# amzn/pecos

Measured on NVIDIA H100. Metric: XR-Linear top-10 queries/sec, higher is better.
Workload: dtype f32

## Files before the change

### pecos_b200/csrc/xlinear_cm_kernel.cuh

```cuda
#pragma once

constexpr int kCmFeat = 8;
constexpr int kCmSlots = 4;
constexpr int kCmMaxWarps = 16;
constexpr int kCmMinWarps = 4;
constexpr uint32_t kCmMaxDup = 400;
constexpr uint32_t kCmSmemBudget = 224u << 10;
constexpr uint32_t kCmMinReuse = 24;
constexpr uint32_t kCmMinPairsPerSm = 48u;
constexpr uint32_t kCmDirectRows = 16384;
constexpr uint32_t kCmEmpty = 0xFFFFFFFFu;

struct CmWork {
    uint32_t* slot_pos;
    uint32_t* count;
    uint32_t* bucket_ptr;
    uint64_t* cost_ptr;
    uint32_t* pair_q;
    uint32_t* pair_pos;
    uint32_t* claim;
    uint32_t* active;
};

struct CmPlan {
// ... 146 lines not shown
            b = rp[r];
            e = rp[r + 1];
            while (b < e && ent[b].x < lo) ++b;
            uint32_t t = b;
            while (t < e && ent[t].x < hi) ++t;
            e = t;
        }
        const uint32_t len = e - b;
        s_scan[threadIdx.x] = len;
        __syncthreads();
        for (uint32_t d = 1; d < 256u; d <<= 1) {
            const uint32_t v = (threadIdx.x >= d) ? s_scan[threadIdx.x - d] : 0u;
            __syncthreads();
            s_scan[threadIdx.x] += v;
            __syncthreads();
        }
        const uint32_t base = s_carry + s_scan[threadIdx.x] - len;
        if (r < R) {
            for (uint32_t i = 0; i < len; ++i) {
                const uint2 en = ent[b + i];
                ec[base + i] = static_cast<unsigned char>(en.x - lo);
                ew[base + i] = __uint_as_float(en.y);
            }
            if (S.direct) {
                unsigned short* starts = reinterpret_cast<unsigned short*>(img + S.off_lookup);
                const uint32_t w_rows = S.words - 1u;
                const uint32_t f = min(ridx[r], w_rows);
                for (uint32_t g = r ? min(ridx[r - 1], w_rows) + 1u : 0u; g <= f; ++g) starts[g] = static_cast<unsigned short>(base);
                if (r + 1u == R)
                    for (uint32_t g = f + 1u; g <= w_rows; ++g) starts[g] = static_cast<unsigned short>(base + len);
            } else {
                rps[r] = static_cast<unsigned short>(base);
            }
            if (r + 1u == R) {
                if (!S.direct) rps[R] = static_cast<unsigned short>(base + len);
                hdr[0] = (h.has_bias & 1u) ? (base | ((base + len) << 16)) : 0u;
                hdr[3] = base + len;
            }
        }
        __syncthreads();
        if (threadIdx.x == 255u) s_carry += s_scan[255];
        __syncthreads();
    }
    if (threadIdx.x == 0) {
        hdr[1] = hi - lo;
        hdr[2] = R;
    }
}

constexpr uint32_t kCmBinWindow = 8192;
constexpr int kCmBucketThreads = 1024;
constexpr uint32_t kCmBucketCtasPerSm = 2;

inline uint32_t cm_bucket_grid(uint32_t rows, uint32_t n_sm) {
    return std::max(1u, std::min(kCmBucketCtasPerSm * n_sm, (rows + kCmBucketThreads / 32 - 1) / (kCmBucketThreads / 32)));
}

struct CmSlotRanges { uint32_t v0, lo, hi, cw; };
__device__ __forceinline__ CmSlotRanges cm_slot_ranges(const uint4 h, const uint32_t* __restrict__ vc_ptr, uint32_t p,
                                                       uint32_t b0, uint32_t nb) {
    CmSlotRanges s{0, 0, 0, 0};
    if ((h.w & kChunkAbsent) || h.y == 0) return s;
    const uint32_t v0 = vc_ptr[p], nr = vc_ptr[p + 1] - v0;
    if (nr == 0) return s;
    s.v0 = v0;
    s.cw = (h.y + nr - 1u) / nr;
    const uint32_t n = min(nr, (h.y + s.cw - 1u) / s.cw);
    s.lo = max(v0, b0);
    s.hi = max(s.lo, min(v0 + n, b0 + nb));
    return s;
}

__device__ __forceinline__ uint2 cm_bucket_block(uint32_t rows) {
    const uint32_t per = (rows + gridDim.x - 1) / gridDim.x;
    const uint32_t b = min(rows, blockIdx.x * per);
    return make_uint2(b, min(rows, b + per));
}

__global__ void __launch_bounds__(kCmBucketThreads, kCmBucketCtasPerSm)
xl_cm_count_kernel(const LayerDev L, const uint32_t* __restrict__ beam_id, const uint32_t* __restrict__ beam_cnt,
                   const uint32_t beam_stride, const uint32_t rows, CmWork w, const uint32_t* __restrict__ vc_ptr,
                   const uint32_t n_vc) {
    __shared__ uint32_t bins[kCmBinWindow];
    const int lane = threadIdx.x & 31, warp = threadIdx.x >> 5, warps = blockDim.x >> 5;
    const uint2 blk = cm_bucket_block(rows);
    for (uint32_t b0 = 0; b0 < n_vc; b0 += kCmBinWindow) {
        const uint32_t nb = min(kCmBinWindow, n_vc - b0);
        for (uint32_t i = threadIdx.x; i < nb; i += blockDim.x) bins[i] = 0u;
        __syncthreads();
        for (uint32_t q = blk.x + warp; q < blk.y; q += warps) {
            const uint32_t cnt = beam_cnt[q];
            uint32_t run = 0;
            for (uint32_t j0 = 0; j0 < cnt; j0 += 32) {
                const uint32_t j = j0 + lane;
                uint4 h = make_uint4(0, 0, 0, kChunkAbsent);
                uint32_t p = 0;
                if (j < cnt) {
                    p = beam_id[static_cast<uint64_t>(q) * beam_stride + j];
                    h = *reinterpret_cast<const uint4*>(&L.chunks[p]);
                }
                if (b0 == 0) {
                    const uint32_t width = (j < cnt) ? h.y : 0u;
                    const uint32_t incl = warp_incl_scan(width, lane);
                    if (j < cnt) w.slot_pos[static_cast<uint64_t>(q) * beam_stride + j] = run + incl - width;
                    run += __shfl_sync(kFull, incl, 31);
                }
                const CmSlotRanges s = cm_slot_ranges(h, vc_ptr, p, b0, nb);
                for (uint32_t v = s.lo; v < s.hi; ++v) atomicAdd(&bins[v - b0], 1u);
            }
        }
        __syncthreads();
        for (uint32_t i = threadIdx.x; i < nb; i += blockDim.x)
            if (bins[i]) atomicAdd(&w.count[b0 + i], bins[i]);
        __syncthreads();
    }
}

__device__ __forceinline__ uint32_t cm_pair_cost(uint32_t w_rows, uint32_t entries) { return w_rows + entries; }

__device__ __forceinline__ uint64_t warp_incl_scan64(uint64_t v, int lane) {
#pragma unroll
    for (int d = 1; d < 32; d <<= 1) {
        const uint64_t t = __shfl_up_sync(kFull, v, d);
        if (lane >= d) v += t;
    }
    return v;
}

__global__ void __launch_bounds__(1024)
xl_cm_scan_kernel(const uint32_t n_chunks, CmWork w, const unsigned char* __restrict__ images, const uint32_t img_bytes,
                  const uint32_t w_rows) {
    __shared__ uint32_t s_pairs[32];
    __shared__ uint64_t s_cost[32];
    __shared__ uint32_t carry_pairs;
    __shared__ uint64_t carry_cost;
    const int lane = threadIdx.x & 31, warp = threadIdx.x >> 5;
    if (threadIdx.x == 0) { carry_pairs = 0; carry_cost = 0; }
    __syncthreads();
    for (uint32_t c0 = 0; c0 < n_chunks; c0 += 1024) {
        const uint32_t c = c0 + threadIdx.x;
        const uint32_t n = (c < n_chunks) ? w.count[c] : 0u;
        const uint32_t unit = n ? cm_pair_cost(w_rows, reinterpret_cast<const uint32_t*>(images + static_cast<uint64_t>(c) * img_bytes)[3]) : 1u;
        const uint64_t cost = static_cast<uint64_t>(n) * unit;
        const uint32_t in_p = warp_incl_scan(n, lane);
        const uint64_t in_c = warp_incl_scan64(cost, lane);
        if (lane == 31) { s_pairs[warp] = in_p; s_cost[warp] = in_c; }
        __syncthreads();
        if (warp == 0) {
            const uint32_t a = s_pairs[lane];
            const uint64_t b = s_cost[lane];
            const uint32_t ia = warp_incl_scan(a, lane);
            const uint64_t ib = warp_incl_scan64(b, lane);
            s_pairs[lane] = ia - a;
            s_cost[lane] = ib - b;
        }
        __syncthreads();
        const uint32_t ex_p = carry_pairs + s_pairs[warp] + in_p - n;
        const uint64_t ex_c = carry_cost + s_cost[warp] + in_c - cost;
        if (c < n_chunks) {
            w.bucket_ptr[c] = ex_p;
            w.cost_ptr[c] = ex_c;
            w.count[c] = ex_p;
            w.claim[c] = ex_p;
            w.active[c] = 0;
        }
        __syncthreads();
        if (threadIdx.x == 1023) { carry_pairs = ex_p + n; carry_cost = ex_c + cost; }
        __syncthreads();
    }
    if (threadIdx.x == 0) { w.bucket_ptr[n_chunks] = carry_pairs; w.cost_ptr[n_chunks] = carry_cost; }
}

__global__ void __launch_bounds__(kCmBucketThreads, kCmBucketCtasPerSm)
xl_cm_scatter_kernel(const LayerDev L, const uint32_t* __restrict__ beam_id, const uint32_t* __restrict__ beam_cnt,
                     const uint32_t beam_stride, const uint32_t rows, CmWork w, const uint32_t* __restrict__ vc_ptr,
                     const uint32_t n_vc) {
    __shared__ uint32_t bins[kCmBinWindow];
    const int lane = threadIdx.x & 31, warp = threadIdx.x >> 5, warps = blockDim.x >> 5;
    const uint2 blk = cm_bucket_block(rows);
    for (uint32_t b0 = 0; b0 < n_vc; b0 += kCmBinWindow) {
        const uint32_t nb = min(kCmBinWindow, n_vc - b0);
        auto each_pair = [&](auto visit) {
            for (uint32_t q = blk.x + warp; q < blk.y; q += warps) {
                const uint32_t cnt = beam_cnt[q];
                for (uint32_t j = lane; j < cnt; j += 32) {
                    const uint32_t p = beam_id[static_cast<uint64_t>(q) * beam_stride + j];
                    const CmSlotRanges s = cm_slot_ranges(*reinterpret_cast<const uint4*>(&L.chunks[p]), vc_ptr, p, b0, nb);
                    if (s.lo < s.hi) visit(q, j, s);
                }
            }
        };
        for (uint32_t i = threadIdx.x; i < nb; i += blockDim.x) bins[i] = 0u;
        __syncthreads();
        each_pair([&](uint32_t, uint32_t, const CmSlotRanges& s) {
            for (uint32_t v = s.lo; v < s.hi; ++v) atomicAdd(&bins[v - b0], 1u);
        });
        __syncthreads();
        for (uint32_t i = threadIdx.x; i < nb; i += blockDim.x)
            if (bins[i]) bins[i] = atomicAdd(&w.count[b0 + i], bins[i]);
        __syncthreads();
        each_pair([&](uint32_t q, uint32_t j, const CmSlotRanges& s) {
            const uint32_t pos = w.slot_pos[static_cast<uint64_t>(q) * beam_stride + j];
            for (uint32_t v = s.lo; v < s.hi; ++v) {
                const uint32_t at = atomicAdd(&bins[v - b0], 1u);
                w.pair_q[at] = q;
                w.pair_pos[at] = pos + (v - s.v0) * s.cw;
            }
        });
        __syncthreads();
    }
}

__device__ inline uint32_t cm_start_chunk(const CmWork& w, uint32_t n_vc, uint32_t b, uint32_t shares) {
    const uint64_t T = w.cost_ptr[n_vc];
    if (T == 0) return n_vc;
    const uint64_t t = static_cast<uint64_t>(T / shares) * b + (T % shares) * b / shares;
    uint32_t lo = 0, hi = n_vc;
    while (hi - lo > 1) {
        const uint32_t mid = (lo + hi) >> 1;
        if (w.cost_ptr[mid] <= t) lo = mid; else hi = mid;
    }
    return lo;
}

enum { kCmPhSwitch, kCmPhCopy, kCmPhStaging, kCmPhLookup, kCmPhAccumulate, kCmPhSlice, kCmPhases };
#ifdef PB200_CM_TRACE
constexpr uint32_t kCmTraceCtas = 1024;
constexpr uint32_t kCmTraceWarp = kCmPhases + 4;
constexpr uint32_t kCmTraceCta = 3 + kCmMaxWarps * kCmTraceWarp;
__device__ unsigned long long g_cm_trace[3 + kCmTraceCtas * kCmTraceCta];
__device__ __forceinline__ unsigned long long cm_globaltimer() {
    unsigned long long t;
    asm volatile("mov.u64 %0, %%globaltimer;" : "=l"(t));
    return t;
}
struct CmTrace {
    unsigned long long start;
    long long t, ph[kCmPhases];
    unsigned long long trips, slots;
    unsigned long long slices, pairs, images;
    __device__ void begin() {
        start = cm_globaltimer();
        t = clock64();
        for (int p = 0; p < kCmPhases; ++p) ph[p] = 0;
        trips = slots = slices = pairs = images = 0;
    }
    __device__ void slice(uint32_t n_pairs) {
        ++slices;
        pairs += n_pairs;
    }
    __device__ void staged() { ++images; }
    __device__ void mark(int p) {
        const long long n = clock64();
        ph[p] += n - t;
        t = n;
    }
    __device__ void count(uint32_t n_trips, uint32_t n_slots) {
        trips += n_trips;
        slots += n_slots;
    }
    __device__ void flush(int warp, int lane, uint32_t launch_pairs) {
        __syncthreads();
        if (blockIdx.x >= kCmTraceCtas) return;
        unsigned long long* rec = g_cm_trace + 3 + blockIdx.x * kCmTraceCta;
        if (threadIdx.x == 0) {
            if (blockIdx.x == 0) { g_cm_trace[0] = gridDim.x; g_cm_trace[1] = blockDim.x >> 5; g_cm_trace[2] = launch_pairs; }
            rec[0] = start;
            rec[1] = cm_globaltimer();
            rec[2] = images;
        }
        for (int d = 16; d > 0; d >>= 1) slots += __shfl_xor_sync(kFull, slots, d);
        if (lane == 0) {
            unsigned long long* wr = rec + 3 + warp * kCmTraceWarp;
            for (int p = 0; p < kCmPhases; ++p) wr[p] = static_cast<unsigned long long>(ph[p]);
            wr[kCmPhases] = trips;
            wr[kCmPhases + 1] = slots;
            wr[kCmPhases + 2] = slices;
            wr[kCmPhases + 3] = pairs;
        }
    }
};
#else
struct CmTrace {
    __device__ void begin() {}
    __device__ void mark(int) {}
    __device__ void count(uint32_t, uint32_t) {}
    __device__ void slice(uint32_t) {}
    __device__ void staged() {}
    __device__ void flush(int, int, uint32_t) {}
};
#endif

template <bool DIRECT, int STAGES, bool PREFIX = false>
__global__ void __launch_bounds__(kCmMaxWarps * 32, 1)
xl_cm_scores_kernel(const LayerDev L, const QueryDev X, const CmWork w, const CmShape S, const unsigned char* __restrict__ images,
                    float* __restrict__ cand, const uint64_t cand_stride_q, const CmPrefixOut P) {
    extern __shared__ __align__(128) unsigned char smem_raw[];
    unsigned char* img = smem_raw;
    const uint32_t* __restrict__ hdr_s = reinterpret_cast<const uint32_t*>(img);
    const unsigned short* __restrict__ start_s = reinterpret_cast<const unsigned short*>(img + S.off_lookup);
    const uint32_t* __restrict__ look_s = reinterpret_cast<const uint32_t*>(img + S.off_lookup);
    const unsigned short* __restrict__ pre_s = reinterpret_cast<const unsigned short*>(img + S.off_pre);
    const unsigned short* __restrict__ rp_s = reinterpret_cast<const unsigned short*>(img + S.off_rp);
    const float* __restrict__ ew_s = reinterpret_cast<const float*>(img + S.off_ew);
    const unsigned char* __restrict__ ec_s = img + S.off_ec;
    const int lane = threadIdx.x & 31;
    const int warp = threadIdx.x >> 5;
    const int nwarps = blockDim.x >> 5;
    constexpr int kStride = kCmFeat + 1;
    constexpr int kBuf = 32 * kStride;
    constexpr int kNBuf = static_cast<int>(cm_buffers(STAGES));
    unsigned char* mine = smem_raw + S.img_bytes + static_cast<size_t>(warp) * cm_warp_bytes(S.acc_cols, STAGES);
    uint32_t* st_idx = reinterpret_cast<uint32_t*>(mine);
    float* st_val = reinterpret_cast<float*>(st_idx + kNBuf * kBuf);
    float* my_acc = st_val + kNBuf * kBuf + lane;

    __shared__ __align__(8) unsigned long long s_mbar;
    const uint32_t mbar = static_cast<uint32_t>(__cvta_generic_to_shared(&s_mbar));
    if (threadIdx.x == 0) {
        cm_mbar_init(mbar, 1u);
        asm volatile("fence.proxy.async.shared::cta;" ::: "memory");
    }
    __syncthreads();
    CmTrace trace;
    trace.begin();

    constexpr int kPerIter = 32 / kCmFeat;
    constexpr int kIters = 32 / kPerIter;
    const int sub = lane / kCmFeat, fl = lane % kCmFeat;
    uint32_t parity = 0;

    uint32_t e = 0, ee = 0, backlog = 0;
    float x = 0.0f;
    uint32_t hp = 0, l1_end = 0;
    auto add_rows = [&](uint32_t row, uint32_t cnt, uint32_t n_ent, bool drain) {
        const uint32_t l2_end = row + cnt;
        const uint32_t avail = backlog + n_ent;
        const uint32_t trips = __reduce_max_sync(kFull, ((drain ? avail : backlog) + kCmSlots - 1u) / kCmSlots);
        if (hp == l1_end) hp = row;
        uint32_t next_r = st_idx[hp];
        float next_x = st_val[hp];
        for (uint32_t t = 0; t < trips; ++t) {
            uint32_t es[kCmSlots], cs[kCmSlots];
            float xs[kCmSlots], a[kCmSlots];
            bool on[kCmSlots];
#pragma unroll
            for (int u = 0; u < kCmSlots; ++u) {
                if (e == ee && hp != l2_end) {
                    e = next_r & 0xFFFFu;
                    ee = next_r >> 16;
                    x = next_x;
                    ++hp;
                    if (hp == l1_end) hp = row;
                    next_r = st_idx[hp];
                    next_x = st_val[hp];
                }
                on[u] = e < ee;
                es[u] = e;
                xs[u] = x;
                e += on[u] ? 1u : 0u;
            }
#pragma unroll
            for (int u = 0; u < kCmSlots; ++u) cs[u] = ec_s[es[u]];
#pragma unroll
            for (int u = 0; u < kCmSlots; ++u) a[u] = my_acc[cs[u] * 32u];
#pragma unroll
            for (int u = 0; u < kCmSlots; ++u) {
                float sum = a[u];
#pragma unroll
                for (int p = 0; p < u; ++p) sum = (cs[p] == cs[u]) ? a[p] : sum;
                a[u] = __fadd_rn(sum, __fmul_rn(xs[u], ew_s[es[u]]));
            }
#pragma unroll
            for (int u = 0; u < kCmSlots; ++u)
                if (on[u]) my_acc[cs[u] * 32u] = a[u];
        }
        const uint32_t added = min(avail, trips * kCmSlots);
        backlog = avail - added;
        trace.count(trips, added);
        l1_end = l2_end;
    };

    uint32_t bias_range = 0, n_cols = 0;
    auto stage_image = [&](uint32_t c) {
        if (threadIdx.x == 0) cm_bulk_load(static_cast<uint32_t>(__cvta_generic_to_shared(img)), images + static_cast<uint64_t>(c) * S.img_bytes, S.img_bytes, mbar);
        cm_mbar_wait(mbar, parity);
        parity ^= 1u;
        trace.staged();
        trace.mark(kCmPhCopy);
        bias_range = hdr_s[0];
        n_cols = hdr_s[1];
    };

    auto score_slice = [&](uint32_t s0, uint32_t s_end) {
        const uint32_t pidx = s0 + lane;
        const bool have = pidx < s_end;
        uint32_t q = 0, pos = 0, qn = 0;
        uint64_t qb = 0;
        if (have) {
            if constexpr (PREFIX) {
                q = pidx;
// ... 218 lines not shown
```

### pecos_b200/csrc/xlinear_engine.cu

```cuda
#include "xlinear_engine.h"
#include "shard_merge.cuh"

#include <algorithm>
#include <atomic>
#include <cstring>
#include <exception>
#include <thread>

namespace pb200 {

namespace {

constexpr unsigned kFull = 0xFFFFFFFFu;
constexpr int kWarpsMax = 10;
constexpr int kMCap = 256;
constexpr int kMFlush = 128;
constexpr int kCSmem = 128;
constexpr int kQCap = 1024;
constexpr int kSortCap = 2048;
constexpr int kTopkThreads = 256;

constexpr int kMCapLookup = 256;

template <int MCAP>
struct __align__(16) WarpScratch {
    uint32_t ms[MCAP];
    float mx[MCAP];
    uint32_t off[MCAP + 4];
    float out[kCSmem];
};

__device__ __forceinline__ uint4 ld_stream_u4(const uint32_t* p) {
    uint4 r;
    asm volatile("ld.global.nc.L1::no_allocate.v4.u32 {%0,%1,%2,%3}, [%4];"
                 : "=r"(r.x), "=r"(r.y), "=r"(r.z), "=r"(r.w) : "l"(p));
    return r;
}

__device__ __forceinline__ int lower_bound_u32(const uint32_t* a, int n, uint32_t key) {
    int lo = 0, hi = n;
    while (lo < hi) {
        int mid = (lo + hi) >> 1;
        if (a[mid] < key) lo = mid + 1; else hi = mid;
    }
    return lo;
}

__device__ __forceinline__ int last_le_u32(const uint32_t* a, int n, uint32_t key) {
    int lo = 0, hi = n;
    while (hi - lo > 1) {
        int mid = (lo + hi) >> 1;
        if (a[mid] <= key) lo = mid; else hi = mid;
    }
    return lo;
}

__device__ __forceinline__ uint32_t warp_incl_scan(uint32_t v, int lane) {
#pragma unroll
    for (int d = 1; d < 32; d <<= 1) {
        uint32_t t = __shfl_up_sync(kFull, v, d);
        if (lane >= d) v += t;
    }
    return v;
}

__device__ __forceinline__ int xl_rows_of_group(const uint32_t* off, int m, uint32_t G, int& row_first, int lane) {
    const int r = row_first + 1 + lane;
    uint32_t bit = 0;
    if (r < m) {
        const uint32_t p = off[r] - G;
        if (p < 32u) bit = 1u << p;
    }
    const uint32_t starts = __reduce_or_sync(kFull, bit);
    const int my_row = row_first + __popc(starts & (0xFFFFFFFFu >> (31 - lane)));
    const int r31 = __shfl_sync(kFull, my_row, 31);
    row_first = (off[r31 + 1] == G + 32u) ? r31 + 1 : r31;
    return my_row;
}

template <int MCAP>
__device__ __forceinline__ void xl_flush_impl(WarpScratch<MCAP>& ws, int m, const uint2* __restrict__ ext,
                                              const uint2* __restrict__ ent, float* out, int lane,
                                              unsigned long long& e_total) {
    if (m == 0) return;
    __syncwarp();
    constexpr int PER = MCAP / 32;
    uint32_t c[PER];
    uint32_t local = 0;
    bool empty_row = false;
#pragma unroll
// ... 288 lines not shown
        }
        __syncwarp();
        if (in_smem) {
            for (uint32_t c = lane; c < h.n_cols; c += 32) blk[c] = ws.out[c];
        }
        __syncwarp();
        if (STATS) { st_chunks += 1; st_rows += R; st_match += m_total; st_ent += e_total; st_cols += h.n_cols; }
    }
    if (STATS) {
        if (lane == 0 && st_chunks) {
            atomicAdd(&stats[0], st_chunks);
            atomicAdd(&stats[1], st_rows);
            atomicAdd(&stats[2], st_match);
            atomicAdd(&stats[3], st_ent);
            atomicAdd(&stats[4], st_cols);
        }
        if (threadIdx.x == 0 && cnt > 0) atomicAdd(&stats[5], static_cast<unsigned long long>(DENSE ? X.cols : qn));
    }
}

__device__ __forceinline__ double xl_hinge_pow(float v, int p) {
    const double zd = fmax(0.0, 1.0 - static_cast<double>(v));
    const float z = static_cast<float>(zd);
    const double x = static_cast<double>(z);
    switch (p) {
        case 0: return 1.0;
        case 1: return x;
        case 2: return x * x;
        case 3: return (x * x) * x;
        case 4: { const double x2 = x * x; return x2 * x2; }
        default: return pow(x, static_cast<double>(static_cast<size_t>(static_cast<long long>(p))));
    }
}

__device__ __forceinline__ float xl_transform(float v, int kind, int p) {
    switch (kind) {
        case PP_SIGMOID: {
            const float e = static_cast<float>(exp(static_cast<double>(-v)));
            return static_cast<float>(1.0 / (1.0 + static_cast<double>(e)));
        }
        case PP_LOG_SIGMOID: {
            const float e = static_cast<float>(exp(static_cast<double>(-v)));
            return static_cast<float>(-log(1.0 + static_cast<double>(e)));
        }
        case PP_LP_HINGE: return static_cast<float>(exp(-xl_hinge_pow(v, p)));
        case PP_LOG_LP_HINGE: return static_cast<float>(-xl_hinge_pow(v, p));
        default: return v;
    }
}

__device__ __forceinline__ float xl_combine(float x, float parent, int kind) {
    switch (kind) {
        case PP_SIGMOID:
        case PP_LP_HINGE: return __fmul_rn(x, parent);
        case PP_LOG_SIGMOID:
        case PP_LOG_LP_HINGE: return __fadd_rn(x, parent);
        default: return x;
    }
}

__device__ __forceinline__ unsigned long long xl_make_key(float v, uint32_t pos) {
    uint32_t u = __float_as_uint(v);
    if ((u & 0x7FFFFFFFu) == 0u) u = 0u;
    u = (u & 0x80000000u) ? ~u : (u | 0x80000000u);
    return (static_cast<unsigned long long>(u) << 32) | static_cast<unsigned long long>(0xFFFFFFFFu - pos);
}

__device__ __forceinline__ unsigned long long xl_exact_key(float v, uint32_t pos) {
    uint32_t u = __float_as_uint(v);
    const uint32_t neg_zero = (u == 0x80000000u) ? 1u : 0u;
    if ((u & 0x7FFFFFFFu) == 0u) u = 0u;
    u = (u & 0x80000000u) ? ~u : (u | 0x80000000u);
    return (static_cast<unsigned long long>(u) << 32) | static_cast<unsigned long long>(0xFFFFFFFFu - ((pos << 1) | neg_zero));
}
__device__ __forceinline__ uint32_t xl_exact_key_pos(unsigned long long key) {
    return (0xFFFFFFFFu - static_cast<uint32_t>(key & 0xFFFFFFFFull)) >> 1;
}
__device__ __forceinline__ float xl_exact_key_value(unsigned long long key) {
    const uint32_t hi = static_cast<uint32_t>(key >> 32);
    const uint32_t bits = (hi & 0x80000000u) ? (hi ^ 0x80000000u) : ~hi;
    return __uint_as_float(((0xFFFFFFFFu - static_cast<uint32_t>(key & 0xFFFFFFFFull)) & 1u) ? 0x80000000u : bits);
}

#include "xlinear_qw_kernel.cuh"
#include "xlinear_cm_kernel.cuh"

__device__ void xl_bitonic_desc(unsigned long long* a, uint32_t n) {
    for (uint32_t k = 2; k <= n; k <<= 1) {
        for (uint32_t j = k >> 1; j > 0; j >>= 1) {
            for (uint32_t i = threadIdx.x; i < n; i += blockDim.x) {
                const uint32_t ixj = i ^ j;
                if (ixj > i) {
                    const unsigned long long x = a[i], y = a[ixj];
                    const bool desc_block = ((i & k) == 0);
                    if (desc_block ? (x < y) : (x > y)) { a[i] = y; a[ixj] = x; }
                }
            }
            __syncthreads();
        }
    }
}

__device__ __forceinline__ uint32_t next_pow2_u32(uint32_t v) {
    if (v <= 2) return 2;
    return 1u << (32 - __clz(v - 1));
}

__global__ void __launch_bounds__(kTopkThreads)
xl_topk_kernel(const LayerDev L, const int pp_kind, const int pp_p, const int combine, const uint32_t k,
               const uint32_t* __restrict__ beam_id, const float* __restrict__ beam_val,
               const uint32_t* __restrict__ beam_cnt, const uint32_t beam_stride, const float* __restrict__ cand,
               const uint64_t cand_stride_q, const uint32_t c_stride, uint32_t* __restrict__ out_id,
               float* __restrict__ out_val, uint32_t* __restrict__ out_cnt, const uint32_t out_stride,
               unsigned long long* sortbuf, const uint64_t sortbuf_stride, const uint32_t b_prev,
               unsigned long long* stats, unsigned long long* __restrict__ out_key) {
    extern __shared__ __align__(16) unsigned char smem_raw[];
    unsigned long long* keys = reinterpret_cast<unsigned long long*>(smem_raw);
    uint32_t* s_base = reinterpret_cast<uint32_t*>(smem_raw + kSortCap * 8);
    uint32_t* s_colbeg = s_base + (b_prev + 1);
    float* s_pval = reinterpret_cast<float*>(s_colbeg + b_prev);

    const uint32_t q = blockIdx.x;
    const uint32_t cnt = beam_cnt[q];
    for (uint32_t j = threadIdx.x; j < cnt; j += blockDim.x) {
        const uint32_t p = beam_id[static_cast<uint64_t>(q) * beam_stride + j];
        const ChunkHeader h = L.chunks[p];
        s_base[j + 1] = h.n_cols;
        s_colbeg[j] = (h.has_bias & kChunkAbsent) ? 0xFFFFFFFFu : h.col_begin;
        s_pval[j] = beam_val[static_cast<uint64_t>(q) * beam_stride + j];
    }
    __syncthreads();
    __shared__ uint32_t s_owned;
    if (threadIdx.x == 0) {
        uint32_t run = 0, owned = 0;
        s_base[0] = 0;
        for (uint32_t j = 0; j < cnt; ++j) {
            if (s_colbeg[j] != 0xFFFFFFFFu) owned += s_base[j + 1];
            run += s_base[j + 1];
            s_base[j + 1] = run;
        }
        s_owned = owned;
    }
    __syncthreads();
    const uint32_t n_valid = s_base[cnt];
    const uint32_t kk = min(k, s_owned);
    if (threadIdx.x == 0) {
        out_cnt[q] = kk;
        if (stats) atomicAdd(&stats[6], static_cast<unsigned long long>(kk));
    }
    if (n_valid == 0) return;

    const float* cq = cand + static_cast<uint64_t>(q) * cand_stride_q;
    auto score_at = [&](uint32_t cpos, uint32_t& label) -> float {
        const uint32_t j = static_cast<uint32_t>(last_le_u32(s_base, static_cast<int>(cnt), cpos));
        const uint32_t off = cpos - s_base[j];
        float v = xl_transform(cq[cpos], pp_kind, pp_p);
        if (combine) v = xl_combine(v, s_pval[j], pp_kind);
        label = s_colbeg[j] + off;
        return v;
    };
    auto key_at = [&](uint32_t cpos) -> unsigned long long {
        const uint32_t j = static_cast<uint32_t>(last_le_u32(s_base, static_cast<int>(cnt), cpos));
        if (s_colbeg[j] == 0xFFFFFFFFu) return 0ull;
        uint32_t lab;
        return xl_make_key(score_at(cpos, lab), cpos);
    };
// ... 529 lines not shown
        b_prev = plan[d].k_cap;
    }
    return plan;
}

uint32_t XLinearEngine::ensure_workspace_(const std::vector<LayerPlan>& plan, uint32_t rows, uint32_t dense_cols) {
    uint64_t beam_stride = 1, cand_max = 1, sort_max = 0, b_max = 1, chunks_max = 1;
    for (size_t d = 0; d < plan.size(); ++d) {
        const uint64_t c = static_cast<uint64_t>(plan[d].b_prev) * std::max<uint32_t>(host_->layers[d].c_max, 1u);
        cand_max = std::max(cand_max, c);
        beam_stride = std::max<uint64_t>(beam_stride, std::max<uint32_t>(plan[d].k_cap, plan[d].b_prev));
        if (c > static_cast<uint64_t>(kSortCap) && plan[d].k > static_cast<uint32_t>(kSortCap / 2)) sort_max = std::max<uint64_t>(sort_max, next_pow2_host(c));
        b_max = std::max<uint64_t>(b_max, plan[d].b_prev);
        chunks_max = std::max<uint64_t>(chunks_max, host_->layers[d].n_chunks);
    }
    const bool cm = chunk_major_ && has_feature_maps();
    const uint64_t pairs = b_max * 4;
    const uint64_t per_query = 16 + 2 * beam_stride * 8 + cand_max * 4 + sort_max * 8 + (cm ? beam_stride * 4 + pairs * 8 : 0);
    uint64_t budget = 8ull << 30;
    if (const char* env = std::getenv("PB200_WORKSPACE_MB")) budget = std::max<uint64_t>(64, std::strtoull(env, nullptr, 10)) << 20;
    uint64_t tile = std::min<uint64_t>(std::max<uint64_t>(1, budget / per_query), std::max<uint32_t>(rows, 1u));
    if (dense_cols) tile = std::min<uint64_t>(tile, std::max<uint64_t>(1, (4ull << 30) / (static_cast<uint64_t>(dense_cols) * 4)));

    beam_stride_ = static_cast<uint32_t>(beam_stride);
    for (int b = 0; b < 2; ++b) {
        beam_id_[b].reserve(tile * beam_stride);
        beam_val_[b].reserve(tile * beam_stride);
        beam_cnt_[b].reserve(tile);
    }
    if (cm) {
        cm_slot_pos_.reserve(tile * beam_stride);
        cm_pair_q_.reserve(tile * pairs);
        cm_pair_pos_.reserve(tile * pairs);
        cm_count_.reserve(chunks_max * 4 + 1);
        cm_claim_.reserve(chunks_max * 4 + 1);
        cm_active_.reserve(chunks_max * 4 + 1);
        cm_bucket_ptr_.reserve(chunks_max * 4 + 1);
        cm_cost_ptr_.reserve(chunks_max * 4 + 1);
    }
    cand_.reserve(tile * cand_max);
    if (sort_max) sortbuf_.reserve(tile * sort_max);
    return static_cast<uint32_t>(tile);
}

int XLinearEngine::score_layer_(size_t d, const QueryDev& q, uint32_t b_prev, int cur, uint32_t ws_row, bool collect_stats) {
    const LayerDev& L = layers_[d].view;
    const uint32_t rows = q.rows;
    const bool dense = (q.row_ptr == nullptr);
    const uint32_t c_stride = std::max<uint32_t>(L.c_max, 1u);
    const uint64_t cand_stride_q = static_cast<uint64_t>(b_prev) * c_stride;
    float* cand = cand_.get() + ws_row * cand_stride_q;
    const uint32_t* bid = bid_(cur, ws_row);
    const uint32_t* bcnt = bcnt_(cur, ws_row);
    unsigned long long* stats = collect_stats ? stats_dev_.get() + 8 * d : nullptr;
    const uint32_t rounds = (b_prev + kWarpsMax - 1) / kWarpsMax;
    const int warps = static_cast<int>(std::max<uint32_t>(1, (b_prev + rounds - 1) / std::max<uint32_t>(rounds, 1)));
    const dim3 grid(rows), block(warps * 32);
    const bool lookup = !dense && L.featmap != nullptr;
    const uint32_t q_cap = dense ? 32u : std::min<uint32_t>(kQCap, std::max<uint32_t>(32u, (q.max_row_nnz + 31u) & ~31u));
    const uint32_t sb_cap = (b_prev + 1u + 3u) & ~3u;
    const uint32_t hdr_cap = b_prev <= 128u ? b_prev : 0u;
    const size_t smem1 = chunk_kernel_smem(warps, lookup, q_cap, sb_cap, hdr_cap);
    auto launch = [&](auto kernel) {
        kernel<<<grid, block, smem1, stream_>>>(L, q, bid, bcnt, beam_stride_, cand,
                                               cand_stride_q, c_stride, stats, q_cap, sb_cap, hdr_cap);
    };
    const bool qw_eligible = lookup && b_prev <= static_cast<uint32_t>(kQwSlots) &&
                             cand_stride_q <= static_cast<uint64_t>(kQwNCap) && q.max_row_nnz <= kQwQCap;
    const bool query_warp = qw_eligible && !no_query_warp_ &&
                            (force_query_warp_ || (b_prev >= 16u && cand_stride_q <= 256u));
    const bool cm_offsets_fit = static_cast<uint64_t>(rows) * std::max<uint32_t>(q.max_row_nnz, 1u) < (1ull << 32);
    const CmPlan cm = (chunk_major_ && lookup && !collect_stats && cm_offsets_fit && cm_slot_pos_.capacity() && layers_[d].cm_images.capacity())
                          ? cm_plan(layers_[d].cm_shape, L.n_chunks, static_cast<uint64_t>(rows) * b_prev, n_sm_, cm_force_)
                          : CmPlan{};
    const bool chunk_major = cm.eligible;
    if (chunk_major) {
        const CmShape& shape = layers_[d].cm_shape;
        const uint32_t n_vc = shape.n_vc;
        CmWork w{cm_slot_pos_.get(), cm_count_.get(), cm_bucket_ptr_.get(), cm_cost_ptr_.get(), cm_pair_q_.get(), cm_pair_pos_.get(),
                 cm_claim_.get(), cm_active_.get()};
        PB200_CUDA(cudaMemsetAsync(w.count, 0, (static_cast<uint64_t>(n_vc) + 1) * 4, stream_));
        const uint32_t bucket_grid = cm_bucket_grid(rows, n_sm_);
        xl_cm_count_kernel<<<bucket_grid, kCmBucketThreads, 0, stream_>>>(L, bid, bcnt, beam_stride_, rows, w, shape.vc_ptr, n_vc);
        xl_cm_scan_kernel<<<1, 1024, 0, stream_>>>(n_vc, w, layers_[d].cm_images.get(), shape.img_bytes, L.w_rows);
        xl_cm_scatter_kernel<<<bucket_grid, kCmBucketThreads, 0, stream_>>>(L, bid, bcnt, beam_stride_, rows, w, shape.vc_ptr, n_vc);
        auto launch_cm = [&](auto kernel) {
            kernel<<<cm.grid, cm.warps * 32, cm.smem, stream_>>>(L, q, w, shape, layers_[d].cm_images.get(), cand, cand_stride_q,
                                                                 CmPrefixOut{});
        };
        if (shape.direct) { if (shape.stages == 4) launch_cm(xl_cm_scores_kernel<true, 4>); else launch_cm(xl_cm_scores_kernel<true, 2>); }
        else { if (shape.stages == 4) launch_cm(xl_cm_scores_kernel<false, 4>); else launch_cm(xl_cm_scores_kernel<false, 2>); }
        launches_ += 3;
    } else if (query_warp) {
        const uint32_t qw_qcap = std::max<uint32_t>(32u, (q.max_row_nnz + 31u) & ~31u);
        const uint32_t qw_ncap = static_cast<uint32_t>((cand_stride_q + 31) & ~static_cast<uint64_t>(31));
        const size_t qw_smem = kQwWarps * ((qw_warp_bytes(qw_qcap, qw_ncap) + 15) & ~static_cast<size_t>(15));
        const dim3 qw_grid((rows + kQwWarps - 1) / kQwWarps);
        if (collect_stats)
            xl_query_warp_scores_kernel<true><<<qw_grid, kQwWarps * 32, qw_smem, stream_>>>(
                L, q, bid, bcnt, beam_stride_, cand, cand_stride_q, stats, qw_qcap, qw_ncap, rows);
        else
            xl_query_warp_scores_kernel<false><<<qw_grid, kQwWarps * 32, qw_smem, stream_>>>(
                L, q, bid, bcnt, beam_stride_, cand, cand_stride_q, stats, qw_qcap, qw_ncap, rows);
    } else if (dense) {
        if (collect_stats) launch(xl_chunk_scores_kernel<true, true, false>);
        else launch(xl_chunk_scores_kernel<true, false, false>);
    } else if (lookup) {
        if (collect_stats) launch(xl_chunk_scores_kernel<false, true, true>);
        else launch(xl_chunk_scores_kernel<false, false, true>);
    } else {
        if (collect_stats) launch(xl_chunk_scores_kernel<false, true, false>);
        else launch(xl_chunk_scores_kernel<false, false, false>);
    }
    PB200_CUDA(cudaGetLastError());
    ++launches_;
    layer_profile_[d].scores_kernel = chunk_major ? 4 : query_warp ? 3 : dense ? 2 : lookup ? 1 : 0;
    return layer_profile_[d].scores_kernel;
}

bool XLinearEngine::use_prefix_(const QueryDev& q, const std::vector<LayerPlan>& plan) const {
    if (!prefix_.cm_shape.ok || !chunk_major_ || no_prefix_ || q.row_ptr == nullptr || !layers_[0].view.featmap || plan.size() < 2)
        return false;
    if (plan[0].k < host_->layers[0].n_cols) return false;
    if (static_cast<uint64_t>(q.rows) * std::max<uint32_t>(q.max_row_nnz, 1u) >= (1ull << 32)) return false;
    return cm_force_ || q.rows >= kCmMinPairsPerSm * n_sm_;
}

void XLinearEngine::launch_prefix_(const QueryDev& q, const std::vector<LayerPlan>& plan, uint32_t ws_row) {
    const CmShape& S = prefix_.cm_shape;
    const uint32_t rows = q.rows;
    const uint32_t grid = std::min<uint32_t>(n_sm_, (rows + 31u) / 32u);
    const uint32_t share = (rows + grid - 1) / grid;
    const uint32_t warps = std::max<uint32_t>(1u, std::min<uint32_t>(S.warps_fit, (share + 31u) / 32u));
    const size_t smem = S.img_bytes + warps * cm_warp_bytes(S.acc_cols, S.stages) + 64;
    CmPrefixOut P;
    P.rows = rows;
    P.n0 = host_->layers[0].n_cols;
    P.pp_kind = plan[0].pp.kind;
    P.pp_p = plan[0].pp.p;
    P.chunks1 = layers_[1].view.chunks;
    P.beam_id = bid_(1, ws_row);
    P.beam_val = bval_(1, ws_row);
    P.beam_cnt = bcnt_(1, ws_row);
    P.beam_stride = beam_stride_;
    P.cand1_stride = static_cast<uint64_t>(plan[1].b_prev) * std::max<uint32_t>(layers_[1].view.c_max, 1u);
    P.cand1 = cand_.get() + ws_row * P.cand1_stride;
    auto launch = [&](auto kernel) {
        kernel<<<grid, warps * 32, smem, stream_>>>(prefix_.view, q, CmWork{}, S, prefix_.cm_images.get(), nullptr, 0, P);
    };
    if (S.stages == 4) launch(xl_cm_scores_kernel<true, 4, true>);
    else launch(xl_cm_scores_kernel<true, 2, true>);
    PB200_CUDA(cudaGetLastError());
    ++launches_;
}

void XLinearEngine::run_tile_(const QueryDev& q, const std::vector<LayerPlan>& plan, const OutTarget& out, uint32_t ws_row,
                              bool collect_stats, bool ext_beam, int combine_first, size_t d_begin, size_t d_end) {
    const uint32_t rows = q.rows;
    if (rows == 0) return;
    int cur = static_cast<int>(d_begin & 1);
    const size_t depth = plan.size();
    d_end = std::min(d_end, depth);
    const bool prefix = !ext_beam && d_begin == 0 && d_end >= 2 && combine_first == 0 && !collect_stats && use_prefix_(q, plan);
    if (!ext_beam && d_begin == 0 && !prefix) {
        xl_init_beam_kernel<<<(rows + 255) / 256, 256, 0, stream_>>>(bid_(cur, ws_row), bval_(cur, ws_row),
                                                                     bcnt_(cur, ws_row), beam_stride_, rows);
        ++launches_;
    }
    for (size_t d = d_begin; d < d_end; ++d) {
        if (prefix && d == 0) {
            if (profile_) PB200_CUDA(cudaEventRecord(ev_[0], stream_));
            launch_prefix_(q, plan, ws_row);
            layer_profile_[0].scores_kernel = 4;
            if (profile_) {
                PB200_CUDA(cudaEventRecord(ev_[1], stream_));
                PB200_CUDA(cudaEventSynchronize(ev_[1]));
                float a = 0.f;
                PB200_CUDA(cudaEventElapsedTime(&a, ev_[0], ev_[1]));
                layer_profile_[0].scores_ms += a;
                layer_profile_[0].launches += 1;
            }
            cur ^= 1;
            continue;
        }
        const LayerDev& L = layers_[d].view;
        const LayerPlan& lp = plan[d];
        const int combine = (d == 0) ? combine_first : 1;
        const uint32_t c_stride = std::max<uint32_t>(L.c_max, 1u);
        const uint64_t cand_stride_q = static_cast<uint64_t>(lp.b_prev) * c_stride;
        const float* cand = cand_.get() + ws_row * cand_stride_q;
        const uint32_t* bid = bid_(cur, ws_row);
        const float* bval = bval_(cur, ws_row);
        const uint32_t* bcnt = bcnt_(cur, ws_row);
        unsigned long long* stats = collect_stats ? stats_dev_.get() + 8 * d : nullptr;
        if (profile_) PB200_CUDA(cudaEventRecord(ev_[0], stream_));
        const dim3 grid(rows);
        const bool scored = prefix && d == 1;
        if (scored) layer_profile_[1].scores_kernel = 4;
        else score_layer_(d, q, lp.b_prev, cur, ws_row, collect_stats);
        if (profile_) PB200_CUDA(cudaEventRecord(ev_[1], stream_));

        const OutTarget o = (d + 1 == depth) ? out
                                             : OutTarget{bid_(cur ^ 1, ws_row), bval_(cur ^ 1, ws_row), bcnt_(cur ^ 1, ws_row),
                                                         nullptr, beam_stride_};
        const uint64_t sort_stride = next_pow2_host(cand_stride_q);
        const bool warp_select = !force_block_topk_ && lp.b_prev <= static_cast<uint32_t>(kSelSlots) &&
                                 cand_stride_q <= static_cast<uint64_t>(kSelKeysMax) && lp.k <= static_cast<uint32_t>(kSelK);
        const bool hinge = lp.pp.kind == PP_LP_HINGE || lp.pp.kind == PP_LOG_LP_HINGE;
        const bool filter_select = !force_block_topk_ && !no_topk_filter_ && lp.k <= 32u &&
                                   lp.b_prev <= static_cast<uint32_t>(kFltSlots) &&
                                   cand_stride_q <= static_cast<uint64_t>(kFltKeysMax) &&
                                   (!hinge || (lp.pp.p >= 0 && lp.pp.p <= 4));
        if (filter_select) {
            const uint32_t key_cap = static_cast<uint32_t>((cand_stride_q + 127) & ~static_cast<uint64_t>(127));
            const size_t flt_smem = kFltWarps * flt_warp_bytes(key_cap);
            xl_topk_filter_kernel<<<(rows + kFltWarps - 1) / kFltWarps, kFltWarps * 32, flt_smem, stream_>>>(
                L, lp.pp.kind, lp.pp.p, combine, lp.k, bid, bval, bcnt,
                beam_stride_, cand, cand_stride_q, o.ids, o.vals, o.cnt, o.stride, rows, stats, o.keys, key_cap);
        } else if (warp_select) {
            const uint32_t key_cap = static_cast<uint32_t>((cand_stride_q + 31) & ~static_cast<uint64_t>(31));
            const size_t sel_smem = kSelWarps * ((sel_warp_bytes(key_cap) + 15) & ~static_cast<size_t>(15));
            xl_topk_warp_kernel<<<(rows + kSelWarps - 1) / kSelWarps, kSelWarps * 32, sel_smem, stream_>>>(
                L, lp.pp.kind, lp.pp.p, combine, lp.k, bid, bval, bcnt,
                beam_stride_, cand, cand_stride_q, c_stride, o.ids, o.vals, o.cnt, o.stride, rows, stats, o.keys, key_cap);
        } else {
            xl_topk_kernel<<<grid, kTopkThreads, topk_kernel_smem(lp.b_prev), stream_>>>(
                L, lp.pp.kind, lp.pp.p, combine, lp.k, bid, bval, bcnt,
                beam_stride_, cand, cand_stride_q, c_stride, o.ids, o.vals, o.cnt, o.stride, sortbuf_.get(), sort_stride,
                lp.b_prev, stats, o.keys);
        }
        PB200_CUDA(cudaGetLastError());
        ++launches_;
        layer_profile_[d].topk_kernel = filter_select ? 2 : warp_select ? 1 : 0;
        if (profile_) {
            PB200_CUDA(cudaEventRecord(ev_[2], stream_));
            PB200_CUDA(cudaEventSynchronize(ev_[2]));
            float a = 0.f, b = 0.f;
            PB200_CUDA(cudaEventElapsedTime(&a, ev_[0], ev_[1]));
            PB200_CUDA(cudaEventElapsedTime(&b, ev_[1], ev_[2]));
            if (!scored) layer_profile_[d].scores_ms += a;
            layer_profile_[d].topk_ms += b;
            layer_profile_[d].launches += scored ? 1 : 2;
        }
        cur ^= 1;
    }
}

XLinearEngine::Result XLinearEngine::finish_result_(uint32_t rows, uint32_t stride) {
    out_ids_.reserve(static_cast<uint64_t>(rows) * stride + 1);
    out_vals_.reserve(static_cast<uint64_t>(rows) * stride + 1);
    out_cnt_.reserve(static_cast<uint64_t>(rows) + 1);
    if (rows) {
        PB200_CUDA(cudaMemcpyAsync(out_ids_.get(), res_ids_dev_.get(), static_cast<uint64_t>(rows) * stride * 4, cudaMemcpyDeviceToHost, stream_));
        PB200_CUDA(cudaMemcpyAsync(out_vals_.get(), res_vals_dev_.get(), static_cast<uint64_t>(rows) * stride * 4, cudaMemcpyDeviceToHost, stream_));
        PB200_CUDA(cudaMemcpyAsync(out_cnt_.get(), res_cnt_dev_.get(), static_cast<uint64_t>(rows) * 4, cudaMemcpyDeviceToHost, stream_));
    }
    PB200_CUDA(cudaStreamSynchronize(stream_));
    Result r;
    r.rows = rows;
    r.stride = stride;
    r.out_cols = host_->layers.back().out_cols;
    r.ids = out_ids_.get();
    r.vals = out_vals_.get();
    r.cnt = out_cnt_.get();
    return r;
}

XLinearEngine::OutTarget XLinearEngine::reserve_results_(uint32_t rows, uint32_t stride) {
    res_ids_dev_.reserve(static_cast<uint64_t>(rows) * stride + 1);
    res_vals_dev_.reserve(static_cast<uint64_t>(rows) * stride + 1);
    res_cnt_dev_.reserve(static_cast<uint64_t>(rows) + 1);
    return OutTarget{res_ids_dev_.get(), res_vals_dev_.get(), res_cnt_dev_.get(), nullptr, stride};
}

void XLinearEngine::for_each_tile_(uint32_t tile, const HostMatrix* x, const TileFn& run) {
    const uint32_t rows = x ? x->rows : resident_.rows;
    for (uint32_t r0 = 0; r0 < rows; r0 += tile) {
        const uint32_t tr = std::min(tile, rows - r0);
        QueryDev q = resident_;
        if (!x) {
            q.row_ptr = resident_.row_ptr + r0;
            q.rows = tr;
        } else if (x->dense) {
            x_val_.upload(x->dense + static_cast<uint64_t>(r0) * x->cols, static_cast<uint64_t>(tr) * x->cols, stream_);
            q = QueryDev{nullptr, nullptr, x_val_.get(), 0, tr, x->cols, x->cols};
        } else {
            const uint64_t base = x->row_ptr[r0], end = x->row_ptr[r0 + tr];
            x_row_ptr_.upload(x->row_ptr + r0, static_cast<uint64_t>(tr) + 1, stream_);
            x_col_idx_.upload(x->col_idx + base, end - base, stream_);
            x_val_.upload(x->val + base, end - base, stream_);
            q = QueryDev{x_row_ptr_.get(), x_col_idx_.get(), x_val_.get(), base, tr, x->cols, max_row_nnz(x->row_ptr + r0, tr)};
        }
        run(q, r0);
    }
}

void XLinearEngine::stage_beam_(uint32_t rows, bool with_vals, const BeamFn& fill) {
    PB200_CUDA(cudaStreamSynchronize(stream_));
    const uint64_t n = static_cast<uint64_t>(rows) * beam_stride_;
    beam_id_host_.reserve(n + 1);
    if (with_vals) beam_val_host_.reserve(n + 1);
// ... 425 lines not shown
```

### pecos_b200/csrc/xlinear_topk_filter.cuh

```cuda
#pragma once

constexpr int kFltWarps = 4;
constexpr int kFltSlots = 64;
constexpr uint32_t kFltKeysMax = 8192;
constexpr int kFltRing = 256;

__host__ __device__ inline size_t flt_warp_bytes(uint32_t key_cap) {
    return (static_cast<size_t>(key_cap) * 4 + (kFltSlots + 1 + kFltSlots + kFltSlots) * 4 + kFltRing * 2 + 4 + 15) &
           ~static_cast<size_t>(15);
}

__device__ __forceinline__ float xl_transform_estimate(float v, int kind, int p) {
    switch (kind) {
        case PP_SIGMOID: return __fdividef(1.0f, 1.0f + __expf(-v));
        case PP_LOG_SIGMOID: return v < -20.0f ? v : -log1pf(__expf(-v));
        case PP_LP_HINGE:
        case PP_LOG_LP_HINGE: {
            const float z = fmaxf(0.0f, 1.0f - v);
            float t;
            switch (p) {
                case 0: t = 1.0f; break;
                case 1: t = z; break;
                case 2: t = z * z; break;
                case 3: t = (z * z) * z; break;
                default: { const float z2 = z * z; t = z2 * z2; } break;
            }
            return kind == PP_LP_HINGE ? __expf(-t) : -t;
        }
        default: return v;
    }
}

__device__ __forceinline__ float xl_from_orderable(uint32_t o) {
    return __uint_as_float((o & 0x80000000u) ? (o ^ 0x80000000u) : ~o);
}

__device__ __forceinline__ unsigned long long xl_umax64(unsigned long long a, unsigned long long b) { return a > b ? a : b; }
__device__ __forceinline__ unsigned long long xl_umin64(unsigned long long a, unsigned long long b) { return a < b ? a : b; }

__device__ __forceinline__ unsigned long long xl_warp_sort_desc(unsigned long long key, int lane) {
#pragma unroll
    for (int k = 2; k <= 32; k <<= 1) {
#pragma unroll
        for (int j = k >> 1; j > 0; j >>= 1) {
            const unsigned long long o = __shfl_xor_sync(kFull, key, j);
            const bool desc = (lane & k) == 0;
            const bool lower = (lane & j) == 0;
            key = (lower == desc) ? xl_umax64(key, o) : xl_umin64(key, o);
        }
    }
    return key;
}

__device__ __forceinline__ unsigned long long xl_warp_bitonic_merge_desc(unsigned long long key, int lane) {
#pragma unroll
    for (int j = 16; j > 0; j >>= 1) {
        const unsigned long long o = __shfl_xor_sync(kFull, key, j);
        key = ((lane & j) == 0) ? xl_umax64(key, o) : xl_umin64(key, o);
    }
    return key;
}

__global__ void __launch_bounds__(kFltWarps * 32)
xl_topk_filter_kernel(const LayerDev L, const int pp_kind, const int pp_p, const int combine, const uint32_t k,
                      const uint32_t* __restrict__ beam_id, const float* __restrict__ beam_val,
                      const uint32_t* __restrict__ beam_cnt, const uint32_t beam_stride, const float* __restrict__ cand,
                      const uint64_t cand_stride_q, uint32_t* __restrict__ out_id, float* __restrict__ out_val,
                      uint32_t* __restrict__ out_cnt, const uint32_t out_stride, const uint32_t rows,
                      unsigned long long* stats, unsigned long long* __restrict__ out_key, const uint32_t key_cap) {
    extern __shared__ __align__(16) unsigned char smem_raw[];
    const int lane = threadIdx.x & 31;
    const int warp = threadIdx.x >> 5;
    const uint32_t q = blockIdx.x * kFltWarps + warp;
    if (q >= rows) return;
    unsigned char* slice = smem_raw + warp * flt_warp_bytes(key_cap);
    uint32_t* keys = reinterpret_cast<uint32_t*>(slice);
    uint32_t* s_base = keys + key_cap;
    uint32_t* s_colbeg = s_base + (kFltSlots + 1);
    float* s_pval = reinterpret_cast<float*>(s_colbeg + kFltSlots);
    unsigned short* ring = reinterpret_cast<unsigned short*>(s_pval + kFltSlots);

    const uint32_t cnt = beam_cnt[q];
    uint32_t run = 0, owned = 0;
    for (uint32_t j0 = 0; j0 < cnt; j0 += 32) {
        const uint32_t j = j0 + lane;
        uint32_t w = 0, cb = 0xFFFFFFFFu;
        float pv = 0.0f;
        if (j < cnt) {
            const uint32_t p = beam_id[static_cast<uint64_t>(q) * beam_stride + j];
            const uint4 h = *reinterpret_cast<const uint4*>(&L.chunks[p]);
            pv = beam_val[static_cast<uint64_t>(q) * beam_stride + j];
            w = h.y;
            cb = (h.w & kChunkAbsent) ? 0xFFFFFFFFu : h.x;
        }
        uint32_t incl = w;
#pragma unroll
        for (int d = 1; d < 32; d <<= 1) {
            const uint32_t t = __shfl_up_sync(kFull, incl, d);
            if (lane >= d) incl += t;
        }
        uint32_t mine = (cb != 0xFFFFFFFFu) ? w : 0u;
#pragma unroll
        for (int d = 16; d > 0; d >>= 1) mine += __shfl_xor_sync(kFull, mine, d);
        if (j < cnt) {
            s_base[j + 1] = run + incl;
            s_colbeg[j] = cb;
            s_pval[j] = pv;
        }
        owned += mine;
        run += __shfl_sync(kFull, incl, 31);
    }
    if (lane == 0) s_base[0] = 0;
    __syncwarp();
    const uint32_t n_valid = run;
    const uint32_t kk = min(k, owned);
    if (lane == 0) {
        out_cnt[q] = kk;
        if (stats) atomicAdd(&stats[6], static_cast<unsigned long long>(kk));
    }
    if (n_valid == 0 || kk == 0) return;
    const float* cq = cand + static_cast<uint64_t>(q) * cand_stride_q;
    const uint32_t n_pad = (n_valid + 127u) & ~127u;

    uint32_t mx = 0, slot = 0;
    for (uint32_t i0 = lane; i0 < n_pad; i0 += 256) {
        float r[8];
#pragma unroll
        for (int u = 0; u < 8; ++u) { const uint32_t i = i0 + 32u * u; r[u] = (i < n_valid) ? cq[i] : 0.0f; }
#pragma unroll
        for (int u = 0; u < 8; ++u) {
            const uint32_t i = i0 + 32u * u;
            uint32_t key = 0;
            if (i < n_valid) {
                while (i >= s_base[slot + 1]) ++slot;
                if (s_colbeg[slot] != 0xFFFFFFFFu) {
                    float s = xl_transform_estimate(r[u], pp_kind, pp_p);
                    if (combine) s = xl_combine(s, s_pval[slot], pp_kind);
                    key = max(orderable(s), 1u);
                }
            }
            if (i < n_pad) keys[i] = key;
            mx = max(mx, key);
        }
    }
    uint32_t tkey = 0;
    {
        uint32_t m = mx;
        for (uint32_t r = 0; r < kk; ++r) {
            tkey = __reduce_max_sync(kFull, m);
            if (tkey == 0) break;
            const int w = __ffs(__ballot_sync(kFull, m == tkey)) - 1;
            if (lane == w) m = 0;
        }
// ... 66 lines not shown
```

Baseline: 23.66 million.

## Launch chained XR-Linear kernels with programmatic dependent launch

Adds griddepcontrol wait and launch-dependents calls at the start of the cm count, scan, scatter, scores and top-k filter kernels. The host now launches the scan, scatter, scores and filter kernels through cudaLaunchKernelEx with programmatic stream serialization. The aim is to hide kernel launch and prologue latency across the short dependent kernel chain. Because each kernel waits immediately, the only overlap is launch setup. Dependents that launch early can occupy SM resources while the previous grid is still running.

```diff
diff --git a/pecos_b200/csrc/xlinear_cm_kernel.cuh b/pecos_b200/csrc/xlinear_cm_kernel.cuh
--- a/pecos_b200/csrc/xlinear_cm_kernel.cuh
+++ b/pecos_b200/csrc/xlinear_cm_kernel.cuh
@@ -252,6 +252,8 @@
                    const uint32_t beam_stride, const uint32_t rows, CmWork w, const uint32_t* __restrict__ vc_ptr,
                    const uint32_t n_vc) {
     __shared__ uint32_t bins[kCmBinWindow];
+    pdl_wait();
+    pdl_allow_dependents();
     const int lane = threadIdx.x & 31, warp = threadIdx.x >> 5, warps = blockDim.x >> 5;
     const uint2 blk = cm_bucket_block(rows);
     for (uint32_t b0 = 0; b0 < n_vc; b0 += kCmBinWindow) {
@@ -304,6 +306,8 @@
     __shared__ uint64_t s_cost[32];
     __shared__ uint32_t carry_pairs;
     __shared__ uint64_t carry_cost;
+    pdl_wait();
+    pdl_allow_dependents();
     const int lane = threadIdx.x & 31, warp = threadIdx.x >> 5;
     if (threadIdx.x == 0) { carry_pairs = 0; carry_cost = 0; }
     __syncthreads();
@@ -346,6 +350,8 @@
                      const uint32_t beam_stride, const uint32_t rows, CmWork w, const uint32_t* __restrict__ vc_ptr,
                      const uint32_t n_vc) {
     __shared__ uint32_t bins[kCmBinWindow];
+    pdl_wait();
+    pdl_allow_dependents();
     const int lane = threadIdx.x & 31, warp = threadIdx.x >> 5, warps = blockDim.x >> 5;
     const uint2 blk = cm_bucket_block(rows);
     for (uint32_t b0 = 0; b0 < n_vc; b0 += kCmBinWindow) {
@@ -487,6 +493,8 @@
 
     __shared__ __align__(8) unsigned long long s_mbar;
     const uint32_t mbar = static_cast<uint32_t>(__cvta_generic_to_shared(&s_mbar));
+    pdl_wait();
+    pdl_allow_dependents();
     if (threadIdx.x == 0) {
         cm_mbar_init(mbar, 1u);
         asm volatile("fence.proxy.async.shared::cta;" ::: "memory");
diff --git a/pecos_b200/csrc/xlinear_engine.cu b/pecos_b200/csrc/xlinear_engine.cu
--- a/pecos_b200/csrc/xlinear_engine.cu
+++ b/pecos_b200/csrc/xlinear_engine.cu
@@ -6,6 +6,7 @@
 #include <cstring>
 #include <exception>
 #include <thread>
+#include <utility>
 
 namespace pb200 {
 
@@ -460,6 +461,23 @@
     return __uint_as_float(((0xFFFFFFFFu - static_cast<uint32_t>(key & 0xFFFFFFFFull)) & 1u) ? 0x80000000u : bits);
 }
 
+__device__ __forceinline__ void pdl_wait() { asm volatile("griddepcontrol.wait;" ::: "memory"); }
+__device__ __forceinline__ void pdl_allow_dependents() { asm volatile("griddepcontrol.launch_dependents;" ::: "memory"); }
+template <typename... Params, typename... Args>
+void launch_pdl(void (*kernel)(Params...), dim3 grid, dim3 block, size_t smem, cudaStream_t stream, Args&&... args) {
+    cudaLaunchAttribute attr[1];
+    attr[0].id = cudaLaunchAttributeProgrammaticStreamSerialization;
+    attr[0].val.programmaticStreamSerializationAllowed = 1;
+    cudaLaunchConfig_t cfg{};
+    cfg.gridDim = grid;
+    cfg.blockDim = block;
+    cfg.dynamicSmemBytes = smem;
+    cfg.stream = stream;
+    cfg.attrs = attr;
+    cfg.numAttrs = 1;
+    PB200_CUDA(cudaLaunchKernelEx(&cfg, kernel, std::forward<Args>(args)...));
+}
+
 #include "xlinear_qw_kernel.cuh"
 #include "xlinear_cm_kernel.cuh"
 
@@ -1155,11 +1173,11 @@
         PB200_CUDA(cudaMemsetAsync(w.count, 0, (static_cast<uint64_t>(n_vc) + 1) * 4, stream_));
         const uint32_t bucket_grid = cm_bucket_grid(rows, n_sm_);
         xl_cm_count_kernel<<<bucket_grid, kCmBucketThreads, 0, stream_>>>(L, bid, bcnt, beam_stride_, rows, w, shape.vc_ptr, n_vc);
-        xl_cm_scan_kernel<<<1, 1024, 0, stream_>>>(n_vc, w, layers_[d].cm_images.get(), shape.img_bytes, L.w_rows);
-        xl_cm_scatter_kernel<<<bucket_grid, kCmBucketThreads, 0, stream_>>>(L, bid, bcnt, beam_stride_, rows, w, shape.vc_ptr, n_vc);
+        launch_pdl(xl_cm_scan_kernel, 1, 1024, 0, stream_, n_vc, w, layers_[d].cm_images.get(), shape.img_bytes, L.w_rows);
+        launch_pdl(xl_cm_scatter_kernel, bucket_grid, kCmBucketThreads, 0, stream_, L, bid, bcnt, beam_stride_, rows, w, shape.vc_ptr, n_vc);
         auto launch_cm = [&](auto kernel) {
-            kernel<<<cm.grid, cm.warps * 32, cm.smem, stream_>>>(L, q, w, shape, layers_[d].cm_images.get(), cand, cand_stride_q,
-                                                                 CmPrefixOut{});
+            launch_pdl(kernel, cm.grid, cm.warps * 32, cm.smem, stream_, L, q, w, shape, layers_[d].cm_images.get(), cand,
+                       cand_stride_q, CmPrefixOut{});
         };
         if (shape.direct) { if (shape.stages == 4) launch_cm(xl_cm_scores_kernel<true, 4>); else launch_cm(xl_cm_scores_kernel<true, 2>); }
         else { if (shape.stages == 4) launch_cm(xl_cm_scores_kernel<false, 4>); else launch_cm(xl_cm_scores_kernel<false, 2>); }
@@ -1219,7 +1237,8 @@
     P.cand1_stride = static_cast<uint64_t>(plan[1].b_prev) * std::max<uint32_t>(layers_[1].view.c_max, 1u);
     P.cand1 = cand_.get() + ws_row * P.cand1_stride;
     auto launch = [&](auto kernel) {
-        kernel<<<grid, warps * 32, smem, stream_>>>(prefix_.view, q, CmWork{}, S, prefix_.cm_images.get(), nullptr, 0, P);
+        launch_pdl(kernel, grid, warps * 32, smem, stream_, prefix_.view, q, CmWork{}, S, prefix_.cm_images.get(), nullptr,
+                   static_cast<uint64_t>(0), P);
     };
     if (S.stages == 4) launch(xl_cm_scores_kernel<true, 4, true>);
     else launch(xl_cm_scores_kernel<true, 2, true>);
@@ -1287,9 +1306,9 @@
         if (filter_select) {
             const uint32_t key_cap = static_cast<uint32_t>((cand_stride_q + 127) & ~static_cast<uint64_t>(127));
             const size_t flt_smem = kFltWarps * flt_warp_bytes(key_cap);
-            xl_topk_filter_kernel<<<(rows + kFltWarps - 1) / kFltWarps, kFltWarps * 32, flt_smem, stream_>>>(
-                L, lp.pp.kind, lp.pp.p, combine, lp.k, bid, bval, bcnt,
-                beam_stride_, cand, cand_stride_q, o.ids, o.vals, o.cnt, o.stride, rows, stats, o.keys, key_cap);
+            launch_pdl(xl_topk_filter_kernel, (rows + kFltWarps - 1) / kFltWarps, kFltWarps * 32, flt_smem, stream_,
+                       L, lp.pp.kind, lp.pp.p, combine, lp.k, bid, bval, bcnt,
+                       beam_stride_, cand, cand_stride_q, o.ids, o.vals, o.cnt, o.stride, rows, stats, o.keys, key_cap);
         } else if (warp_select) {
             const uint32_t key_cap = static_cast<uint32_t>((cand_stride_q + 31) & ~static_cast<uint64_t>(31));
             const size_t sel_smem = kSelWarps * ((sel_warp_bytes(key_cap) + 15) & ~static_cast<size_t>(15));
diff --git a/pecos_b200/csrc/xlinear_topk_filter.cuh b/pecos_b200/csrc/xlinear_topk_filter.cuh
--- a/pecos_b200/csrc/xlinear_topk_filter.cuh
+++ b/pecos_b200/csrc/xlinear_topk_filter.cuh
@@ -69,6 +69,8 @@
                       uint32_t* __restrict__ out_cnt, const uint32_t out_stride, const uint32_t rows,
                       unsigned long long* stats, unsigned long long* __restrict__ out_key, const uint32_t key_cap) {
     extern __shared__ __align__(16) unsigned char smem_raw[];
+    pdl_wait();
+    pdl_allow_dependents();
     const int lane = threadIdx.x & 31;
     const int warp = threadIdx.x >> 5;
     const uint32_t q = blockIdx.x * kFltWarps + warp;
```

Result: faster. 23.92 million (median of 6 runs) (+1.1%).
